# gitMasterLiujiahui/AlphaZero-Gomoku

Hardware: AMD Instinct MI355X
Metric: self-play moves/sec at 200 sims/move, 15x15 board, 1/2/4/8 MI355X (higher is better)
Workload: dtype f16x3 (fp32-equivalent split, f32 accumulate); tree forward: root children as a delta of the root's fp32 accumulators, within 2e-5 of the full forward and 1e-4 of the reference (tests/test_gpu_pvdelta.py)

## Files before the change

### alphazero-gomoku_amd/csrc/gz_pvdg.hip

```cpp
#include <hip/hip_runtime.h>

#include <cstdlib>

#include "gz_internal.h"
#include "gz_pvtree.h"

using namespace gzpv;

namespace {

using namespace gzc;

constexpr int NTD = 256;
#ifndef GZ_DG_NTE
#define GZ_DG_NTE 1
#endif
__host__ __device__ constexpr int dg_s(int L) { return 2 * L + 3; }
__host__ __device__ constexpr int dg_ss(int L) { return dg_s(L) * dg_s(L); }
__host__ __device__ constexpr int dg_so(int L) { return 2 * L + 5; }

__host__ __device__ constexpr int dgk_g(int L) { return L == 0 ? 6 : (L == 1 ? 3 : (L == 2 ? 2 : 1)); }
__host__ __device__ constexpr int dgk_npos(int L) { return (dgk_g(L) * dg_ss(L) + 1 + 15) & ~15; }
struct K {
    static constexpr int C = 6;
    __host__ __device__ static constexpr int g(int L) { return dgk_g(L); }
    static constexpr int NPASS = 1 + C / 3 + C / 2 + C;
    __host__ __device__ static constexpr int pass_of(int L, int gi) {
        return L == 0 ? 0 : (L == 1 ? 1 + gi / 3 : (L == 2 ? 3 + 3 * (gi / 2) : 4 + 3 * (gi / 2) + (gi & 1)));
    }
    __host__ __device__ static constexpr int npos(int L) { return dgk_npos(L); }
    static constexpr int MAXNPOS = 112;
    static constexpr int NMAX = 12;
    static constexpr int ROWS = NMAX * 16;
    static constexpr int GB = 2;
    static constexpr int WPS = 2;
    static constexpr int NKEY = 36;
    static constexpr int IN = 0;
    static constexpr int IN_BYTES = 32 * MAXNPOS * 16;
    static constexpr int COL = 32 * dgk_npos(0) * 16;
    static constexpr int HP = IN + IN_BYTES;
    static constexpr int HP_BYTES = dgk_g(3) * 4 * 3 * 121 * 4;
    static constexpr int ROWT = HP + HP_BYTES;
    static constexpr int MASK = ROWT + NPASS * ROWS * 4;
    static constexpr int HIST = MASK + NPASS * 16 * 4;
    static constexpr int U = HIST + 2 * NPASS * NKEY * 4;
    static constexpr int CST = U + C * 128;
    static constexpr int CST_FLOATS = 4 * 128 + 3 * 128 + 4;
    static constexpr int POS = CST + CST_FLOATS * 4;
    static constexpr int LDS = POS + 16;
};
static_assert(dgk_npos(0) <= K::MAXNPOS && dgk_npos(1) <= K::MAXNPOS && dgk_npos(2) == K::MAXNPOS &&
                  dgk_npos(3) <= K::MAXNPOS, "image");
static_assert(K::LDS * K::WPS <= 160 * 1024, "LDS budget");
static_assert(K::COL + K::C * 1024 <= K::IN_BYTES, "im2col behind the y1 image");
static_assert(dgk_g(0) * dg_so(0) * dg_so(0) <= K::ROWS && dgk_g(1) * dg_so(1) * dg_so(1) <= K::ROWS &&
                  dgk_g(2) * dg_so(2) * dg_so(2) <= K::ROWS && dgk_g(3) * dg_so(3) * dg_so(3) <= K::ROWS, "rows");
static_assert(K::C % 6 == 0 && dgk_g(3) == 1, "passes; one x2 node per pass (the record prefetch)");
static_assert(K::C == 6 && dgk_g(1) == 3 && dgk_g(2) == 2, "pass order (K::pass_of, dg_pass_of): 2 x1 triples, 3 y2 pairs");

__host__ __device__ constexpr int scr_sq(int map, int node) {
    return (map == 0 ? 9 * node : (map == 2 ? 54 + 49 * node : (map == 1 ? 348 + (node >= 3 ? 25 * (node - 3) : 0) : 348))) * 256;
}
constexpr int SCR_HALVES = (348 + 81) * 256;
static_assert(348 + 3 * 25 <= 348 + 81 && 54 + 49 * 6 == 348, "scratch regions");

struct DgUnit {
    const _Float16* gm;
    const float* pre;
    _Float16* own;
    _Float16* patch;
    int leaf, base, cell, pad0;
    int sq[4];
    uint32_t board[16];
};
static_assert(sizeof(DgUnit) == 128, "unit size");

struct DgArgs {
    const int32_t* cinfo;
    const float* W;
    const uint32_t* boards;
    const int32_t* meta;
    const int32_t* pslot;
    const _Float16* maps;
    const float* pres;
    _Float16* patches;
    float* hbuf;
    int32_t* tiles;
    int32_t* queue;
};

#ifdef GZ_PVDG_STAMPS
__device__ unsigned long long gz_pvdg_stamps[16];
__device__ unsigned long long gz_pvdg_stamps_n[1];
using DgStamp = PhaseStamp<gz_pvdg_stamps>;
#else
using DgStamp = PhaseStamp<nullptr>;
#endif

#define GZ_GLB __attribute__((address_space(1)))
#ifdef GZ_DG_CHK
__device__ unsigned long long gz_dg_chk[16];
__device__ const char* gz_dg_lo;
__device__ const char* gz_dg_hi;
__device__ __forceinline__ const void* dg_chk(const void* p, int code) {
    if ((const char*)p < gz_dg_lo || (const char*)p >= gz_dg_hi) {
        atomicAdd(&gz_dg_chk[code], 1ull);
        return gz_dg_lo;
    }
    return p;
}
#define DG_CHK(p, code) dg_chk((p), (code))
#else
#define DG_CHK(p, code) (p)
#endif
template <class T>
__device__ __forceinline__ T gld(const void* p) {
    return *(const GZ_GLB T*)DG_CHK(p, 0);
}
template <class T>
__device__ __forceinline__ void gst(void* p, const T& v) {
    *(GZ_GLB T*)DG_CHK(p, 1) = v;
}

__device__ __forceinline__ int set_rank(int b) {
    return b == 7 ? 0 : (b == 3 ? 1 : (b == 1 ? 2 : (b == 6 ? 3 : (b == 2 ? 4 : 5))));
}

__device__ __forceinline__ void dg_rows_all(char* lds, const DgUnit* U, int ng, int tid) {
    uint32_t* hist = (uint32_t*)(lds + K::HIST);
    uint32_t* starts = hist + K::NPASS * K::NKEY;
    uint32_t* rt0 = (uint32_t*)(lds + K::ROWT);
    uint32_t* mk0 = (uint32_t*)(lds + K::MASK);
    constexpr int N0 = 25, N1 = 49, N2 = 81, N3 = 121;
    const int o1 = ng * N0, o2 = o1 + ng * N1, o3 = o2 + ng * N2, tot = o3 + ng * N3;
    constexpr int PER = (K::C * (N0 + N1 + N2 + N3) + NTD - 1) / NTD;
    int kk[PER], rank[PER];
    uint32_t ent[PER];
#pragma unroll
    for (int i = 0; i < PER; i++) {
        const int c = tid + i * NTD;
        kk[i] = -1;
        rank[i] = 0;
        ent[i] = 0;
        if (c >= tot) continue;
        const int L = c < o1 ? 0 : (c < o2 ? 1 : (c < o3 ? 2 : 3));
        const int SO = 2 * L + 5, RO = L + 2, RIN = L + 1;
        const int cl = c - (L == 0 ? 0 : (L == 1 ? o1 : (L == 2 ? o2 : o3)));
        const int gi = cl / (SO * SO), j = cl - gi * (SO * SO), dy = j / SO - RO, dx = j - (j / SO) * SO - RO;
        const int cell = U[gi].cell, cr = cell / BN, cc = cell - (cell / BN) * BN;
        const int pr = cr + dy, pc = cc + dx;
        if (pr < 0 || pr >= BN || pc < 0 || pc >= BN) continue;
        int ty = 0, tx = 0;
#pragma unroll
        for (int d = -1; d <= 1; d++) {
            const int qy = dy + d, qx = dx + d;
            if (qy >= -RIN && qy <= RIN && cr + qy >= 0 && cr + qy < BN) ty |= 1 << (d + 1);
            if (qx >= -RIN && qx <= RIN && cc + qx >= 0 && cc + qx < BN) tx |= 1 << (d + 1);
        }
        if (!ty || !tx) continue;
        uint32_t m = 0;
#pragma unroll
        for (int a = 0; a < 3; a++)
            if ((ty >> a) & 1) m |= (uint32_t)tx << (3 * a);
        const int gl = L == 0 ? 0 : (L == 1 ? 3 : (L == 2 ? 2 : 1));
        const int p = K::pass_of(L, gi), u0 = L == 0 ? 0 : (gi / gl) * gl;
        kk[i] = p * K::NKEY + set_rank(ty) * 6 + set_rank(tx);
        ent[i] = (uint32_t)(gi - u0) | ((uint32_t)(dy + RO) << 4) | ((uint32_t)(dx + RO) << 8) | (m << 12) | (1u << 21);
        rank[i] = (int)atomicAdd(&hist[kk[i]], 1u);
    }
    __syncthreads();
    {
        const int w = tid >> 6, ln = tid & 63;
        for (int p = w; p < K::NPASS; p += NTD / 64) {
            const uint32_t v = ln < K::NKEY ? hist[p * K::NKEY + ln] : 0u;
            uint32_t x = v;
#pragma unroll
            for (int d = 1; d < 64; d <<= 1) {
                const uint32_t y = __shfl_up(x, d);
                if (ln >= d) x += y;
            }
            if (ln < K::NKEY) {
                starts[p * K::NKEY + ln] = x - v;
                hist[p * K::NKEY + ln] = 0u;
            }
            if (ln == 63) mk0[p * 16 + 9] = x;
        }
    }
    __syncthreads();
#pragma unroll
    for (int i = 0; i < PER; i++)
        if (kk[i] >= 0) rt0[(kk[i] / K::NKEY) * K::ROWS + starts[kk[i]] + rank[i]] = ent[i];
    for (int e = tid; e < K::NPASS * K::ROWS; e += NTD)
        if ((uint32_t)(e % K::ROWS) >= mk0[(e / K::ROWS) * 16 + 9]) rt0[e] = 0u;
    __syncthreads();
    {
        const int w = tid >> 6, ln = tid & 63;
        for (int p = w; p < K::NPASS; p += NTD / 64) {
            const uint32_t* rt = rt0 + p * K::ROWS;
            uint32_t tm = 0;
            if (ln < K::NMAX)
#pragma unroll
                for (int k = 0; k < 16; k++) tm |= (rt[ln * 16 + k] >> 12) & 0x1ffu;
            int exec = 0;
#pragma unroll
            for (int t = 0; t < 9; t++) {
                const uint64_t b = __ballot((tm >> t) & 1u);
                if (ln == 0) mk0[p * 16 + t] = (uint32_t)b;
                exec += __popcll(b);
            }
            if (ln == 0) mk0[p * 16 + 10] = (uint32_t)exec;
        }
    }
}

template <int NT, int L>
__device__ __forceinline__ void dg_kloop(const char* lds, const uint32_t (&ri)[K::NMAX], const uint32_t* mk,
                                         const _Float16* __restrict__ Wf, int nt0, int lane,
                                         f32x4 (&acc)[2][K::NMAX]) {
    constexpr int S = dg_s(L), NPOS = K::npos(L), CQ = 4, KS = 9 * CQ;
    constexpr int CQB = 4 * NPOS * 16, PLB = 16 * NPOS * 16, ZIDX = NPOS - 1;
    constexpr int KS_BYTES = 8 * 64 * 8 * 2, LO_BYTES = KS * KS_BYTES, RING = 4;
    const int lb = K::IN + (lane >> 4) * NPOS * 16;
    const __amdgpu_buffer_rsrc_t wr = __builtin_amdgcn_make_buffer_rsrc((void*)Wf, 0, 0x7fffffff, 0x00020000);
    const int wo = (nt0 * 64 + lane) * 16;
    auto wload = [&](int ks, int n, int lo) -> h8 {
        return __builtin_bit_cast(h8, __builtin_amdgcn_raw_buffer_load_b128(wr, wo, ks * KS_BYTES + n * 1024 + lo * LO_BYTES, 0));
    };
    auto addr = [&](int tap, uint32_t r) -> int {
        const int toff = (tap / 3 - 1) * S + (tap - (tap / 3) * 3 - 1);
        const bool v = (r >> (16 + tap)) & 1u;
        return lb + (v ? (int)(r & 0xffffu) - 32 + toff : ZIDX) * 16;
    };
    h8 b[RING][2][2];
#pragma unroll
    for (int c = 0; c < 2; c++)
#pragma unroll
        for (int n = 0; n < 2; n++) {
            b[c][n][0] = wload(c, n, 0);
            b[c][n][1] = wload(c, n, 1);
        }
    f32x4 c[2][NT];
#pragma unroll
    for (int n = 0; n < 2; n++)
#pragma unroll
        for (int m = 0; m < NT; m++) c[n][m] = acc[n][m];
    int ad[NT];
#pragma unroll
    for (int m = 0; m < NT; m++) ad[m] = addr(0, ri[m]);
    h8 fh[2][2], fl[2][2];
#pragma unroll
    for (int k2 = 0; k2 < 2; k2++) {
        fh[0][k2] = *(const h8*)(lds + ad[0] + k2 * CQB);
        fl[0][k2] = *(const h8*)(lds + ad[0] + k2 * CQB + PLB);
    }
#pragma unroll 1
    for (int tap = 0; tap < 9; tap++) {
        const uint32_t tm = (uint32_t)__builtin_amdgcn_readfirstlane((int)mk[tap]);
#pragma unroll
        for (int h = 0; h < 2; h++) {
            {
                const int ksr = tap * CQ + 2 * h + 2;
                const int kn = ksr < KS ? ksr : ksr - KS;
#pragma unroll
                for (int k2 = 0; k2 < 2; k2++)
#pragma unroll
                    for (int n = 0; n < 2; n++) {
                        b[(2 * h + 2 + k2) & 3][n][0] = wload(kn + k2, n, 0);
                        b[(2 * h + 2 + k2) & 3][n][1] = wload(kn + k2, n, 1);
                    }
            }
#pragma unroll
            for (int m = 0; m < NT; m++) {
                const int pm = m & 1, pn = (m + 1) & 1;
                int na;
                if (m + 1 < NT) na = ad[m + 1] + 2 * h * CQB;
                else na = h == 0 ? ad[0] + 2 * CQB : ad[0];
#pragma unroll
                for (int k2 = 0; k2 < 2; k2++) {
                    fh[pn][k2] = *(const h8*)(lds + na + k2 * CQB);
                    fl[pn][k2] = *(const h8*)(lds + na + k2 * CQB + PLB);
                }
                if (h == 1) ad[m] = addr(tap + 1, ri[m]);
                if ((tm >> m) & 1u) {
#pragma unroll
                    for (int k2 = 0; k2 < 2; k2++) {
                        const int sl = 2 * h + k2;
                        const h8 ah = fh[pm][k2], al = fl[pm][k2];
#pragma unroll
                        for (int n = 0; n < 2; n++) c[n][m] = __builtin_amdgcn_mfma_f32_16x16x32_f16(b[sl][n][0], ah, c[n][m], 0, 0, 0);
#pragma unroll
                        for (int n = 0; n < 2; n++) c[n][m] = __builtin_amdgcn_mfma_f32_16x16x32_f16(b[sl][n][1], ah, c[n][m], 0, 0, 0);
#pragma unroll
                        for (int n = 0; n < 2; n++) c[n][m] = __builtin_amdgcn_mfma_f32_16x16x32_f16(b[sl][n][0], al, c[n][m], 0, 0, 0);
                    }
                }
            }
        }
    }
#pragma unroll
    for (int n = 0; n < 2; n++)
#pragma unroll
        for (int m = 0; m < NT; m++) acc[n][m] = c[n][m];
}

struct H4x2 {
    h4 h, l;
};
__device__ __forceinline__ float h2f(const H4x2& x, int r) { return (float)x.h[r] + (float)x.l[r]; }
__device__ __forceinline__ void put_hl(_Float16* p, int plane_halves, const f32x4& v) {
    h4 hi, lo;
#pragma unroll
    for (int r = 0; r < 4; r++) {
        const _Float16 h = (_Float16)v[r];
        hi[r] = h;
        lo[r] = (_Float16)(v[r] - (float)h);
    }
    gst<h4>(p, hi);
    gst<h4>(p + plane_halves, lo);
}
__device__ __forceinline__ void put_hl_lds(_Float16* p, int plane_halves, const f32x4& v) {
    h4 hi, lo;
#pragma unroll
    for (int r = 0; r < 4; r++) {
        const _Float16 h = (_Float16)v[r];
        hi[r] = h;
        lo[r] = (_Float16)(v[r] - (float)h);
    }
    *(h4*)p = hi;
    *(h4*)(p + plane_halves) = lo;
}

template <int L>
__device__ __forceinline__ void dg_epilogue(char* lds, const DgUnit* U, const uint32_t* rt, int np, int lane,
                                            const f32x4 (&acc)[2][K::NMAX], int nt, int ldsg) {
    constexpr int RO = L + 2, SO = dg_so(L), SSO = SO * SO;
    constexpr bool SKIP = L == 1 || L == 3;
    constexpr int RS = L == 1 ? 1 : 3, SK = 2 * RS + 1, SSK = SK * SK;
    constexpr int GB = K::GB, NGRP = (K::NMAX + GB - 1) / GB, ST = 2;
    float* hpart = (float*)(lds + K::HP);
    const int q = lane >> 4, li = lane & 15;
    const float* cst = (const float*)(lds + K::CST);
    f32x4 es[2], e0[2], e1[2], ev[2];
#pragma unroll
    for (int n = 0; n < 2; n++) {
        const int ch0 = (2 * np + n) * 16 + 4 * q;
        es[n] = *(const f32x4*)(cst + L * 128 + ch0);
        if (L == 3) {
            e0[n] = *(const f32x4*)(cst + 512 + ch0);
            e1[n] = *(const f32x4*)(cst + 640 + ch0);
            ev[n] = *(const f32x4*)(cst + 768 + ch0);
        }
    }
    f32x4 z[ST][GB][2];
    H4x2 dk[ST][GB][2];
    uint32_t ent[ST][GB];
    auto loads = [&](int grp, int st) {
#pragma unroll
        for (int j = 0; j < GB; j++) {
            const int m = grp * GB + j;
            if (m >= K::NMAX) break;
            const uint32_t e = rt[m * 16 + li];
            ent[st][j] = e;
            const int gi = e & 15, dy = (int)((e >> 4) & 15) - RO, dx = (int)((e >> 8) & 15) - RO;
            const DgUnit& u = U[gi];
            const int cell = u.cell, cr = cell / BN, cc = cell - (cell / BN) * BN;
            const bool v = (e >> 21) & 1u;
            const int pos = v ? (cr + dy) * BN + (cc + dx) : 0;
            const bool near = SKIP && v && iabs(dy) <= RS && iabs(dx) <= RS;
            const int sidx = near ? (dy + RS) * SK + (dx + RS) : 0;
#pragma unroll
            for (int n = 0; n < 2; n++) {
                const int ch0 = (2 * np + n) * 16 + 4 * q;
                z[st][j][n] = gld<f32x4>(u.pre + L * PV_PRE_FLOATS + pos * CH + ch0);
                if (SKIP) {
                    const _Float16* p = u.own + u.sq[L - 1] + ((ch0 >> 3) * SSK + sidx) * 8 + (ch0 & 7);
                    dk[st][j][n] = H4x2{gld<h4>(p), gld<h4>(p + 16 * SSK * 8)};
                }
            }
        }
    };
#pragma unroll
    for (int grp = 0; grp < ST - 1; grp++)
        if (grp * GB < nt) loads(grp, grp);
#pragma unroll
    for (int grp = 0; grp < NGRP; grp++) {
        if (grp * GB >= nt) break;
        const int st = grp % ST;
        if ((grp + ST - 1) * GB < nt) loads(grp + ST - 1, (grp + ST - 1) % ST);
#pragma unroll
        for (int j = 0; j < GB; j++) {
            const int m = grp * GB + j;
            if (m >= K::NMAX) break;
            const uint32_t e = ent[st][j];
            const bool v = (e >> 21) & 1u;
            const int gi = e & 15, dy = (int)((e >> 4) & 15) - RO, dx = (int)((e >> 8) & 15) - RO;
            const bool near = SKIP && iabs(dy) <= RS && iabs(dx) <= RS;
            const int oidx = (dy + RO) * SO + (dx + RO);
            float s0 = 0.f, s1 = 0.f, sv = 0.f;
#pragma unroll
            for (int n = 0; n < 2; n++) {
                const int ch0 = (2 * np + n) * 16 + 4 * q;
                f32x4 y, d;
#pragma unroll
                for (int r = 0; r < 4; r++) {
                    const float zr = z[st][j][n][r];
                    float tc = __builtin_fmaf(acc[n][m][r], es[n][r], zr);
                    if (SKIP) tc += near ? h2f(dk[st][j][n], r) : 0.f;
                    tc = tc > 0.f ? tc : 0.f;
                    if (L == 3) {
                        s0 = __builtin_fmaf(e0[n][r], tc, s0);
                        s1 = __builtin_fmaf(e1[n][r], tc, s1);
                        sv = __builtin_fmaf(ev[n][r], tc, sv);
                    } else {
                        y[r] = tc;
                        d[r] = tc - (zr > 0.f ? zr : 0.f);
                    }
                }
                if (L < 3 && v) {
                    const DgUnit& u = U[gi];
                    const int o = PATCH_OFF[L + 1] + ((ch0 >> 3) * SSO + oidx) * 8 + (ch0 & 7);
                    if (gi < ldsg) {
                        constexpr int NPN = K::npos(L + 1 < 4 ? L + 1 : 3), SSN = SSO;
                        put_hl_lds((_Float16*)(lds + K::IN) + ((ch0 >> 3) * NPN + gi * SSN + oidx) * 8 + (ch0 & 7),
                                   16 * NPN * 8, d);
                    } else {
                        put_hl(u.own + u.sq[L + 1] + ((ch0 >> 3) * SSO + oidx) * 8 + (ch0 & 7), 16 * SSO * 8, d);
                    }
                    if (u.patch) put_hl(u.patch + o, 16 * SSO * 8, y);
                }
            }
            if (L == 3) {
                s0 += __shfl_xor(s0, 16);
                s1 += __shfl_xor(s1, 16);
                sv += __shfl_xor(sv, 16);
                s0 += __shfl_xor(s0, 32);
                s1 += __shfl_xor(s1, 32);
                sv += __shfl_xor(sv, 32);
                if (lane < 16 && v) {
                    float* h = hpart + ((gi * 4 + np) * 3) * 121 + oidx;
                    h[0] = s0;
                    h[121] = s1;
                    h[242] = sv;
                }
            }
        }
    }
}

constexpr int REC_K = (HSTRIDE + NTD - 1) / NTD;
__device__ __forceinline__ void dg_record_load(const DgUnit& u, const float* __restrict__ hbuf, float (&rec)[REC_K],
                                               int tid) {
    const float* src = (const float*)DG_CHK(hbuf + (size_t)u.base * HSTRIDE, 3);
#pragma unroll
    for (int k = 0; k < REC_K; k++) {
        const int j = tid + k * NTD;
        rec[k] = j < HSTRIDE ? src[j] : 0.f;
    }
}
__device__ __forceinline__ void dg_record(const DgUnit& u, int g, const float* bias, float* __restrict__ hbuf,
                                          const float* hpart, const float (&rec)[REC_K], int tid) {
    const int cr = u.cell / BN, cc = u.cell - (u.cell / BN) * BN;
    float* h = (float*)DG_CHK(hbuf + (size_t)u.leaf * HSTRIDE, 4);
#pragma unroll
    for (int k = 0; k < REC_K; k++) {
        const int j = tid + k * NTD;
        if (j >= HSTRIDE) break;
        float v = rec[k];
        int pos = -1, which = 0;
        if (j < POS) {
            pos = j;
        } else if (j < 2 * POS) {
            pos = j - POS;
            which = 1;
        } else if (j >= HV_OFF && j < HV_OFF + POS) {
            pos = j - HV_OFF;
            which = 2;
        }
        if (pos >= 0) {
            const int dy = pos / BN - cr, dx = pos % BN - cc;
            if (iabs(dy) <= 5 && iabs(dx) <= 5) {
                const int idx = (dy + 5) * 11 + (dx + 5);
                float a = bias[which];
#pragma unroll
                for (int w = 0; w < 4; w++) a += hpart[((g * 4 + w) * 3 + which) * 121 + idx];
                v = a;
            }
        }
        h[j] = v;
    }
}

template <int L>
__device__ __forceinline__ void dg_fill(char* lds, const DgUnit* U, int g, int tid) {
    constexpr int SS = dg_ss(L), NPOS = K::npos(L), NB = (NPOS + 63) / 64;
    const int lane = tid & 63, wave = tid >> 6;
#pragma unroll
    for (int blk = 0; blk < NB; blk++) {
        const int idx = blk * 64 + lane;
        const _Float16* src = (const _Float16*)gz_tree_zero16;
        int stride = 0;
        if (idx < g * SS) {
            const int gi = idx / SS, j = idx - gi * SS;
            src = U[gi].own + U[gi].sq[L] + j * 8;
            stride = SS * 8;
        }
        char* dst = lds + K::IN + blk * 64 * 16;
        if (idx < NPOS) {
#pragma unroll
            for (int k = 0; k < 8; k++) {
                const int pc = wave * 8 + k;
                __builtin_amdgcn_global_load_lds((glb_void_t*)DG_CHK(src + pc * stride, 2), (lds_void_t*)(dst + pc * NPOS * 16),
                                                 16, 0, 0);
            }
        }
    }
}

__device__ __forceinline__ void dg_col(_Float16* col, const DgUnit* U, int ng, int tid) {
    for (int e = tid; e < ng * 512; e += NTD) {
        const int g = e >> 9, row = (e >> 5) & 15, k = e & 31;
        const DgUnit& u = U[g];
        const int cr = u.cell / BN, cc = u.cell - (u.cell / BN) * BN;
        const int r0 = cr > 0 ? cr - 1 : 0, r1 = cr < BN - 1 ? cr + 1 : BN - 1;
        const int c0 = cc > 0 ? cc - 1 : 0, c1 = cc < BN - 1 ? cc + 1 : BN - 1, wr = c1 - c0 + 1;
        _Float16 v = (_Float16)0.f;
        if (row < (r1 - r0 + 1) * wr && k < 27) {
            const int pr = r0 + row / wr, pc = c0 + row % wr;
            const int tap = k / 3, cin = k % 3;
            const int rr = pr + tap / 3 - 1, c2 = pc + tap % 3 - 1;
            if (rr >= 0 && rr < BN && c2 >= 0 && c2 < BN) {
                const int bit = rr * 16 + c2;
                const uint32_t bl = (u.board[bit >> 5] >> (bit & 31)) & 1u, wh = (u.board[8 + (bit >> 5)] >> (bit & 31)) & 1u;
                v = (_Float16)(float)(cin == 0 ? bl : (cin == 1 ? wh : 1u - (bl | wh)));
            }
        }
        col[e] = v;
    }
}

__device__ __forceinline__ void dg_conv0(char* lds, const _Float16* col, const DgUnit* U, int ng,
                                         const float* __restrict__ W, int np, int lane) {
    constexpr int NPOS = K::npos(0);
    const int li = lane & 15, q = lane >> 4;
    h8 wh[2], wl[2];
    f32x4 ws[2], wt[2];
#pragma unroll
    for (int n = 0; n < 2; n++) {
        const int nt = 2 * np + n, ch0 = nt * 16 + 4 * q;
        const _Float16* wf = (const _Float16*)(W + F16_C0) + ((size_t)nt * 64 + lane) * 8;
        wh[n] = *(const h8*)wf;
        wl[n] = *(const h8*)(wf + 8 * 64 * 8);
        ws[n] = *(const f32x4*)(W + C0_S + ch0);
        wt[n] = *(const f32x4*)(W + C0_T + ch0);
    }
    _Float16* in = (_Float16*)(lds + K::IN);
    h4 rxh[K::C][2], rxl[K::C][2];
#pragma unroll
    for (int g = 0; g < K::C; g++) {
        const DgUnit& u = U[g < ng ? g : 0];
        const int cr = u.cell / BN, cc = u.cell - (u.cell / BN) * BN;
        const int r0 = cr > 0 ? cr - 1 : 0, r1 = cr < BN - 1 ? cr + 1 : BN - 1;
        const int c0 = cc > 0 ? cc - 1 : 0, c1 = cc < BN - 1 ? cc + 1 : BN - 1, wr = c1 - c0 + 1;
        const bool rowok = li < (r1 - r0 + 1) * wr;
        const int pr = rowok ? r0 + li / wr : cr, pc = rowok ? c0 + li % wr : cc, pos = pr * BN + pc;
#pragma unroll
        for (int n = 0; n < 2; n++) {
            const int ch0 = (2 * np + n) * 16 + 4 * q;
            const _Float16* rp = u.gm + ((ch0 >> 3) * 256 + pos) * 8 + (ch0 & 7);
            rxh[g][n] = gld<h4>(rp);
            rxl[g][n] = gld<h4>(rp + PV_MAP_PLANE);
        }
    }
#pragma unroll
    for (int g = 0; g < K::C; g++) {
        if (g >= ng) break;
        const h8 a = *(const h8*)(col + g * 512 + li * 32 + 8 * q);
        const DgUnit& u = U[g];
        const int cr = u.cell / BN, cc = u.cell - (u.cell / BN) * BN;
        const int r0 = cr > 0 ? cr - 1 : 0, r1 = cr < BN - 1 ? cr + 1 : BN - 1;
        const int c0 = cc > 0 ? cc - 1 : 0, c1 = cc < BN - 1 ? cc + 1 : BN - 1, wr = c1 - c0 + 1;
        const bool rowok = li < (r1 - r0 + 1) * wr;
        const int pr = rowok ? r0 + li / wr : cr, pc = rowok ? c0 + li % wr : cc;
        const int idx = (pr - cr + 1) * 3 + (pc - cc + 1);
#pragma unroll
        for (int n = 0; n < 2; n++) {
            const int ch0 = (2 * np + n) * 16 + 4 * q;
            f32x4 acc = zero4();
            acc = __builtin_amdgcn_mfma_f32_16x16x32_f16(wh[n], a, acc, 0, 0, 0);
            acc = __builtin_amdgcn_mfma_f32_16x16x32_f16(wl[n], a, acc, 0, 0, 0);
            if (rowok) {
                const h4 rh = rxh[g][n], rl = rxl[g][n];
                f32x4 y, d;
#pragma unroll
                for (int r = 0; r < 4; r++) {
                    float t = __builtin_fmaf(acc[r], ws[n][r], wt[n][r]);
                    t = t > 0.f ? t : 0.f;
                    y[r] = t;
                    d[r] = t - ((float)rh[r] + (float)rl[r]);
                }
                put_hl_lds(in + ((ch0 >> 3) * NPOS + g * 9 + idx) * 8 + (ch0 & 7), 16 * NPOS * 8, d);
                const int o = PATCH_OFF[0] + ((ch0 >> 3) * 9 + idx) * 8 + (ch0 & 7);
                put_hl(u.own + u.sq[0] + o, 16 * 9 * 8, d);
                if (u.patch) put_hl(u.patch + o, 16 * 9 * 8, y);
            }
        }
    }
}

template <int L>
__device__ __forceinline__ void dg_pass(const char* lds, const uint32_t* rt, const uint32_t* mk,
                                        const float* __restrict__ W, int np, int lane, f32x4 (&acc)[2][K::NMAX], int nt) {
    constexpr int RIN = L + 1, RO = L + 2, S = dg_s(L), SS = dg_ss(L);
    const int li = lane & 15;
    uint32_t ri[K::NMAX];
#pragma unroll
    for (int m = 0; m < K::NMAX; m++) {
        const uint32_t e = rt[m * 16 + li];
        const int gi = e & 15, dy = (int)((e >> 4) & 15) - RO, dx = (int)((e >> 8) & 15) - RO;
        const int base = gi * SS + (dy + RIN) * S + (dx + RIN) + 32;
        ri[m] = (e >> 21) & 1u ? ((uint32_t)base & 0xffffu) | (((e >> 12) & 0x1ffu) << 16) : 0u;
    }
#pragma unroll
    for (int n = 0; n < 2; n++)
#pragma unroll
        for (int m = 0; m < K::NMAX; m++) acc[n][m] = zero4();
    const _Float16* Wf = (const _Float16*)(W + F16_RES0 + L * F16_STRIDE);
#if GZ_DG_NTE
    constexpr int MT = (dgk_g(L) * dg_so(L) * dg_so(L) + 15) / 16, MTE = (MT + 1) & ~1;
    static_assert(MTE <= K::NMAX, "tiles");
    const int nte = (nt + 1) & ~1;
    if (nte <= 2)
        dg_kloop<2, L>(lds, ri, mk, Wf, 2 * np, lane, acc);
    else if (nte == 4)
        dg_kloop<4, L>(lds, ri, mk, Wf, 2 * np, lane, acc);
    else if (nte == 6 || MTE <= 6)
        dg_kloop<6 < MTE ? 6 : MTE, L>(lds, ri, mk, Wf, 2 * np, lane, acc);
    else if (nte == 8 || MTE <= 8)
        dg_kloop<8 < MTE ? 8 : MTE, L>(lds, ri, mk, Wf, 2 * np, lane, acc);
    else if (nte == 10 || MTE <= 10)
        dg_kloop<10 < MTE ? 10 : MTE, L>(lds, ri, mk, Wf, 2 * np, lane, acc);
    else
        dg_kloop<MTE, L>(lds, ri, mk, Wf, 2 * np, lane, acc);
#else
    if (nt <= 4)
        dg_kloop<4, L>(lds, ri, mk, Wf, 2 * np, lane, acc);
    else if (nt <= 8)
        dg_kloop<8, L>(lds, ri, mk, Wf, 2 * np, lane, acc);
    else
        dg_kloop<K::NMAX, L>(lds, ri, mk, Wf, 2 * np, lane, acc);
#endif
}

__device__ __forceinline__ void dg_pass_of(int p, int ng, int& L, int& u0, int& g) {
    if (p < 3) {
        L = p == 0 ? 0 : 1;
        u0 = p == 0 ? 0 : (p - 1) * 3;
    } else {
        const int k = (p - 3) / 3, r = p - 3 - 3 * k;
        L = r == 0 ? 2 : 3;
        u0 = 2 * k + (r == 2 ? 1 : 0);
    }
    g = ng - u0 < K::g(L) ? ng - u0 : K::g(L);
    if (L == 0) u0 = 0, g = ng;
}

__global__ __launch_bounds__(NTD, K::WPS) void pv_dg_kernel(DgArgs A, _Float16* __restrict__ scratch,
                                                           const int32_t* __restrict__ list,
                                                           const int32_t* __restrict__ list_count) {
    __shared__ __attribute__((aligned(16))) char lds[K::LDS];
    DgUnit* const U = (DgUnit*)(lds + K::U);
    const int count = *list_count;
    const int nx = gridDim.x >= 8 ? 8 : 1;
    const int xcd = blockIdx.x % nx, per = gridDim.x / nx, k = blockIdx.x / nx;
    if (k >= per) return;
    const int xchunk = (count + nx - 1) / nx;
    int q = 0, claim = 0;
    if (threadIdx.x == 0) claim = atomicAdd(A.queue + xcd, K::C);
    _Float16* myscr = scratch + (size_t)blockIdx.x * SCR_HALVES;
    const int tid = threadIdx.x, lane = tid & 63;
    const int wave = __builtin_amdgcn_readfirstlane(tid >> 6), np = wave;
    const float* W = A.W;
    for (int i = tid; i < K::NPASS * K::NKEY; i += NTD) ((uint32_t*)(lds + K::HIST))[i] = 0u;
    {
        float* cst = (float*)(lds + K::CST);
        for (int i = tid; i < K::CST_FLOATS; i += NTD) {
            float v;
            if (i < 512) v = W[RES0 + (i >> 7) * RES_STRIDE + RES_S + (i & 127)];
            else if (i < 768) v = W[P_W + (i - 512)];
            else if (i < 896) v = W[V_W + (i - 768)];
            else v = i == 896 ? W[P_B] : (i == 897 ? W[P_B + 1] : (i == 898 ? W[V_B] : 0.f));
            cst[i] = v;
        }
    }
    DgStamp st;
    for (;;) {
        __syncthreads();
        if (threadIdx.x == 0) {
            int pb = count, pe = count;
            for (;;) {
                const int qx = (xcd + q) % nx, xb = qx * xchunk, xe = xb + xchunk < count ? xb + xchunk : count;
                if (xb + claim < xe) {
                    pb = xb + claim, pe = xe;
                    claim = atomicAdd(A.queue + qx, K::C);
                    break;
                }
                if (++q == nx) break;
                claim = atomicAdd(A.queue + (xcd + q) % nx, K::C);
            }
            ((int*)(lds + K::POS))[0] = pb;
            ((int*)(lds + K::POS))[1] = pe;
        }
        __syncthreads();
        const int pos = ((const int*)(lds + K::POS))[0], xe = ((const int*)(lds + K::POS))[1];
        if (pos >= xe) break;
        const int ng = xe - pos < K::C ? xe - pos : K::C;
        if (wave == 0 && lane < ng) {
            const int b = list[pos + lane];
            DgUnit u;
            const int ci = A.cinfo[b];
            const int o = (ci >> 8) & 0x3fffff;
            u.gm = A.maps + (size_t)o * 4 * PV_MAP_HALVES;
            u.pre = A.pres + (size_t)o * 4 * PV_PRE_FLOATS;
            u.own = myscr;
            u.sq[0] = scr_sq(0, lane);
            u.sq[1] = scr_sq(1, lane);
            u.sq[2] = scr_sq(2, lane);
            u.sq[3] = scr_sq(3, lane);
            const int ps = A.pslot[b];
            u.patch = ps >= 0 ? A.patches + (size_t)ps * PATCH_HALVES : nullptr;
            u.leaf = b;
            u.base = A.meta[b];
            u.cell = ci & 0xff;
            u.pad0 = 0;
#pragma unroll
            for (int w = 0; w < 16; w++) u.board[w] = A.boards[(size_t)b * 16 + w];
            U[lane] = u;
        }
        __syncthreads();
        {
            int t = tid;
            asm volatile("" : "+v"(t));
            dg_col((_Float16*)(lds + K::COL), U, ng, t);
            constexpr int NPOS0 = K::npos(0);
            const int z0 = ng * 9;
            for (int e = t; e < 32 * (NPOS0 - z0); e += NTD) {
                const int pc = e / (NPOS0 - z0), idx = z0 + e % (NPOS0 - z0);
                *(uint4*)(lds + K::IN + (pc * NPOS0 + idx) * 16) = make_uint4(0u, 0u, 0u, 0u);
            }
            __syncthreads();
            const float* Wp = W;
            asm volatile("" : "+s"(Wp));
            dg_conv0(lds, (const _Float16*)(lds + K::COL), U, ng, Wp, np, t & 63);
            dg_rows_all(lds, U, ng, t);
            __syncthreads();
#ifdef GZ_DG_CHK
            for (int e = tid; e < K::NPASS * K::ROWS; e += NTD) {
                const int pp = e / K::ROWS;
                int L_, u0_, g_;
                dg_pass_of(pp, ng, L_, u0_, g_);
                const uint32_t tot = ((const uint32_t*)(lds + K::MASK))[pp * 16 + 9];
                const uint32_t en = ((const uint32_t*)(lds + K::ROWT))[e];
                if ((uint32_t)(e % K::ROWS) < tot && (!((en >> 21) & 1u) || (int)(en & 15) >= g_))
                    atomicAdd(&gz_dg_chk[8], 1ull);
                if ((uint32_t)(e % K::ROWS) >= tot && en != 0u) atomicAdd(&gz_dg_chk[9], 1ull);
            }
            if (tid < K::C && (U[tid].cell < 0 || U[tid].cell >= 225) && tid < ng) atomicAdd(&gz_dg_chk[10], 1ull);
#endif
        }
        st(0);
#ifdef GZ_PVDG_STAMPS
        if (blockIdx.x == 0 && threadIdx.x == 0) atomicAdd(&gz_pvdg_stamps_n[0], (unsigned long long)ng);
#endif
        for (int p = 0; p < K::NPASS; p++) {
            int L, u0, g;
            dg_pass_of(p, ng, L, u0, g);
            if (g <= 0) continue;
            const uint32_t* rt = (const uint32_t*)(lds + K::ROWT) + p * K::ROWS;
            const uint32_t* mk = (const uint32_t*)(lds + K::MASK) + p * 16;
            const int nrows = (int)mk[9], nt = (nrows + 15) >> 4;
            if (A.tiles && tid == 0) atomicAdd(A.tiles, (int)mk[10]);
            const float* Wp = W;
            int t = tid;
            asm volatile("" : "+s"(Wp), "+v"(t));
#ifdef GZ_DG_CHK
            for (int e = tid; e < K::ROWS; e += NTD) {
                const uint32_t en = rt[e];
                if ((uint32_t)e < (uint32_t)nrows && (!((en >> 21) & 1u) || (int)(en & 15) >= g))
                    atomicAdd(&gz_dg_chk[11 + (L > 1 ? 1 : 0)], 1ull);
            }
#endif
            f32x4 acc[2][K::NMAX];
            if (L == 0) dg_pass<0>(lds, rt, mk, Wp, np, t & 63, acc, nt);
            else if (L == 1) dg_pass<1>(lds, rt, mk, Wp, np, t & 63, acc, nt);
            else if (L == 2) dg_pass<2>(lds, rt, mk, Wp, np, t & 63, acc, nt);
            else dg_pass<3>(lds, rt, mk, Wp, np, t & 63, acc, nt);
            st(2 + L);
            __syncthreads();
            st(6);
            int q = p + 1, L2 = 0, v0 = 0, g2 = 0;
            for (; q < K::NPASS; q++) {
                dg_pass_of(q, ng, L2, v0, g2);
                if (g2 > 0) break;
            }
            const bool more = q < K::NPASS;
            const int ldsg = more && L2 == L + 1 && v0 == u0 && (L == 0 || L == 2) ? g2 : 0;
            const bool to_lds = ldsg > 0;
            if (L == 0) dg_epilogue<0>(lds, U + u0, rt, np, t & 63, acc, nt, ldsg);
            else if (L == 1) dg_epilogue<1>(lds, U + u0, rt, np, t & 63, acc, nt, 0);
            else if (L == 2) dg_epilogue<2>(lds, U + u0, rt, np, t & 63, acc, nt, ldsg);
            else dg_epilogue<3>(lds, U + u0, rt, np, t & 63, acc, nt, 0);
            if (to_lds) {
                const int NPN = L == 0 ? K::npos(1) : K::npos(3), z0 = ldsg * (L == 0 ? dg_ss(1) : dg_ss(3));
                for (int e = t; e < 32 * (NPN - z0); e += NTD) {
                    const int pc = e / (NPN - z0), idx = z0 + e % (NPN - z0);
                    *(uint4*)(lds + K::IN + (pc * NPN + idx) * 16) = make_uint4(0u, 0u, 0u, 0u);
                }
            }
            st(7 + L);
            const bool reads_mine = more && !to_lds && L2 == L + 1 && v0 < u0 + g && u0 < v0 + g2;
            if (reads_mine) asm volatile("s_waitcnt vmcnt(0)" ::: "memory");
            if (reads_mine || L == 3) __syncthreads();
            st(11);
            if (more && !to_lds) {
                if (L2 == 1) dg_fill<1>(lds, U + v0, g2, t);
                else if (L2 == 2) dg_fill<2>(lds, U + v0, g2, t);
                else if (L2 == 3) dg_fill<3>(lds, U + v0, g2, t);
            }
            if (L == 3) {
                float rec[REC_K];
                dg_record_load(U[u0], A.hbuf, rec, t);
                dg_record(U[u0], 0, (const float*)(lds + K::CST) + 896, A.hbuf, (const float*)(lds + K::HP), rec, t);
                asm volatile("s_waitcnt vmcnt(2)" ::: "memory");
            } else {
                asm volatile("s_waitcnt vmcnt(0)" ::: "memory");
            }
            st(12);
            __syncthreads();
            st(13);
        }
    }
}

}

int gz_internal_tree_delta(const TreeWs& t, const float* d_weights, const uint32_t* d_boards, const int32_t* d_meta,
                           int grid, void* stream) {
    DgArgs A{t.cinfo, d_weights, d_boards, d_meta, t.pslot, t.maps, t.pres, t.patches, t.hbuf,
             t.ctr + CTR_TILES, t.ctr + CTR_DG_QUEUE};
    static_assert(K::WPS * SCR_HALVES <= PV_SCRATCH_PATCHES * PATCH_HALVES, "scratch");
#ifdef GZ_PVDG_STAMPS
    static const int wps = std::getenv("GZ_PVDG_WPS") && std::getenv("GZ_PVDG_WPS")[0] == '1' ? 1 : K::WPS;
#else
    constexpr int wps = K::WPS;
#endif
#ifdef GZ_DG_CHK
    {
        const char* lo = (const char*)t.hbuf;
        const char* hi = (const char*)(t.scratch + (size_t)grid * PV_SCRATCH_PATCHES * PATCH_HALVES);
        hipMemcpyToSymbolAsync(HIP_SYMBOL(gz_dg_lo), &lo, sizeof(lo), 0, hipMemcpyHostToDevice, (hipStream_t)stream);
        hipMemcpyToSymbolAsync(HIP_SYMBOL(gz_dg_hi), &hi, sizeof(hi), 0, hipMemcpyHostToDevice, (hipStream_t)stream);
    }
#endif
    pv_dg_kernel<<<grid * wps, NTD, 0, (hipStream_t)stream>>>(A, t.scratch, t.children, t.ctr + CTR_CHILDREN);
    return gz_check_launch("tree delta");
}

#ifdef GZ_PVDG_STAMPS
extern "C" int gz_pvdg_stamps_read(unsigned long long* out, int reset) {
    if (hipMemcpyFromSymbol(out, HIP_SYMBOL(gz_pvdg_stamps), 16 * sizeof(unsigned long long)) != hipSuccess) return -1;
    if (hipMemcpyFromSymbol(out + 16, HIP_SYMBOL(gz_pvdg_stamps_n), sizeof(unsigned long long)) != hipSuccess) return -1;
    if (reset) {
        unsigned long long z[16] = {0};
        if (hipMemcpyToSymbol(HIP_SYMBOL(gz_pvdg_stamps), z, sizeof(z)) != hipSuccess) return -1;
        if (hipMemcpyToSymbol(HIP_SYMBOL(gz_pvdg_stamps_n), z, sizeof(z[0])) != hipSuccess) return -1;
    }
    return 0;
}
#endif

#ifdef GZ_DG_CHK
extern "C" int gz_pvdg_chk_read(unsigned long long* out) {
    if (hipDeviceSynchronize() != hipSuccess) return -1;
    return hipMemcpyFromSymbol(out, HIP_SYMBOL(gz_dg_chk), 16 * sizeof(unsigned long long)) == hipSuccess ? 0 : -1;
}
#endif
```

Measured before the change: 37150.

## Remap MFMA output channels so each lane owns 8 contiguous channels

```diff
diff --git a/alphazero-gomoku_amd/csrc/gz_dgclass.h b/alphazero-gomoku_amd/csrc/gz_dgclass.h
--- /dev/null
+++ b/alphazero-gomoku_amd/csrc/gz_dgclass.h
@@ -0,0 +1,32 @@
+#pragma once
+
+#ifdef __HIPCC__
+#define GZ_DGCLASS_FN __host__ __device__ constexpr
+#else
+#define GZ_DGCLASS_FN constexpr
+#endif
+
+GZ_DGCLASS_FN int dg_set_rank(int b) {
+    return b == 1 ? 0 : (b == 3 ? 1 : (b == 7 ? 2 : (b == 6 ? 3 : (b == 4 ? 4 : 5))));
+}
+GZ_DGCLASS_FN bool dg_set_valid(int b) { return b == 1 || b == 3 || b == 7 || b == 6 || b == 4 || b == 2; }
+
+GZ_DGCLASS_FN int dg_class_rank(int ty, int tx) {
+    const int ry = dg_set_rank(ty), rx = dg_set_rank(tx);
+    return ry * 6 + ((ry & 1) ? 5 - rx : rx);
+}
+
+GZ_DGCLASS_FN bool dg_class_rank_is_permutation() {
+    unsigned long long seen = 0;
+    for (int ty = 1; ty < 8; ty++)
+        for (int tx = 1; tx < 8; tx++) {
+            if (!dg_set_valid(ty) || !dg_set_valid(tx)) continue;
+            const int k = dg_class_rank(ty, tx);
+            if (k < 0 || k >= 36 || ((seen >> k) & 1ull)) return false;
+            seen |= 1ull << k;
+        }
+    return seen == (1ull << 36) - 1ull;
+}
+static_assert(dg_class_rank_is_permutation(), "the 36 valid (ty, tx) pairs map onto 0..35 exactly once");
+
+#undef GZ_DGCLASS_FN
diff --git a/alphazero-gomoku_amd/csrc/gz_pvdg.hip b/alphazero-gomoku_amd/csrc/gz_pvdg.hip
--- a/alphazero-gomoku_amd/csrc/gz_pvdg.hip
+++ b/alphazero-gomoku_amd/csrc/gz_pvdg.hip
@@ -2,6 +2,7 @@
 
 #include <cstdlib>
 
+#include "gz_dgclass.h"
 #include "gz_internal.h"
 #include "gz_pvtree.h"
 
@@ -122,9 +123,13 @@
     *(GZ_GLB T*)DG_CHK(p, 1) = v;
 }
 
-__device__ __forceinline__ int set_rank(int b) {
-    return b == 7 ? 0 : (b == 3 ? 1 : (b == 1 ? 2 : (b == 6 ? 3 : (b == 2 ? 4 : 5))));
-}
+__device__ __forceinline__ int dg_ch0(int np, int q, int n) { return 32 * np + 8 * q + 4 * n; }
+__device__ __forceinline__ int dg_wfrag(int np, int lane) {
+    const int i = lane & 15;
+    return (2 * np + (i >> 3)) * 64 + ((lane & 48) | (8 * ((i >> 2) & 1) + (i & 3)));
+}
+constexpr int DG_WFRAG_N = 4;
+
 
 __device__ __forceinline__ void dg_rows_all(char* lds, const DgUnit* U, int ng, int tid) {
     uint32_t* hist = (uint32_t*)(lds + K::HIST);
@@ -164,7 +169,7 @@
             if ((ty >> a) & 1) m |= (uint32_t)tx << (3 * a);
         const int gl = L == 0 ? 0 : (L == 1 ? 3 : (L == 2 ? 2 : 1));
         const int p = K::pass_of(L, gi), u0 = L == 0 ? 0 : (gi / gl) * gl;
-        kk[i] = p * K::NKEY + set_rank(ty) * 6 + set_rank(tx);
+        kk[i] = p * K::NKEY + dg_class_rank(ty, tx);
         ent[i] = (uint32_t)(gi - u0) | ((uint32_t)(dy + RO) << 4) | ((uint32_t)(dx + RO) << 8) | (m << 12) | (1u << 21);
         rank[i] = (int)atomicAdd(&hist[kk[i]], 1u);
     }
@@ -222,9 +227,9 @@
     constexpr int KS_BYTES = 8 * 64 * 8 * 2, LO_BYTES = KS * KS_BYTES, RING = 4;
     const int lb = K::IN + (lane >> 4) * NPOS * 16;
     const __amdgpu_buffer_rsrc_t wr = __builtin_amdgcn_make_buffer_rsrc((void*)Wf, 0, 0x7fffffff, 0x00020000);
-    const int wo = (nt0 * 64 + lane) * 16;
+    const int wo = dg_wfrag(nt0 >> 1, lane) * 16;
     auto wload = [&](int ks, int n, int lo) -> h8 {
-        return __builtin_bit_cast(h8, __builtin_amdgcn_raw_buffer_load_b128(wr, wo, ks * KS_BYTES + n * 1024 + lo * LO_BYTES, 0));
+        return __builtin_bit_cast(h8, __builtin_amdgcn_raw_buffer_load_b128(wr, wo, ks * KS_BYTES + n * DG_WFRAG_N * 16 + lo * LO_BYTES, 0));
     };
     auto addr = [&](int tap, uint32_t r) -> int {
         const int toff = (tap / 3 - 1) * S + (tap - (tap / 3) * 3 - 1);
@@ -303,31 +308,29 @@
         for (int m = 0; m < NT; m++) acc[n][m] = c[n][m];
 }
 
-struct H4x2 {
-    h4 h, l;
+struct H8x2 {
+    h8 h, l;
 };
-__device__ __forceinline__ float h2f(const H4x2& x, int r) { return (float)x.h[r] + (float)x.l[r]; }
-__device__ __forceinline__ void put_hl(_Float16* p, int plane_halves, const f32x4& v) {
-    h4 hi, lo;
-#pragma unroll
-    for (int r = 0; r < 4; r++) {
-        const _Float16 h = (_Float16)v[r];
-        hi[r] = h;
-        lo[r] = (_Float16)(v[r] - (float)h);
-    }
-    gst<h4>(p, hi);
-    gst<h4>(p + plane_halves, lo);
-}
-__device__ __forceinline__ void put_hl_lds(_Float16* p, int plane_halves, const f32x4& v) {
-    h4 hi, lo;
-#pragma unroll
-    for (int r = 0; r < 4; r++) {
-        const _Float16 h = (_Float16)v[r];
-        hi[r] = h;
-        lo[r] = (_Float16)(v[r] - (float)h);
-    }
-    *(h4*)p = hi;
-    *(h4*)(p + plane_halves) = lo;
+__device__ __forceinline__ float h2f(const H8x2& x, int r) { return (float)x.h[r] + (float)x.l[r]; }
+__device__ __forceinline__ H8x2 split_hl(const f32x4 (&v)[2]) {
+    H8x2 o;
+#pragma unroll
+    for (int n = 0; n < 2; n++)
+#pragma unroll
+        for (int r = 0; r < 4; r++) {
+            const _Float16 h = (_Float16)v[n][r];
+            o.h[4 * n + r] = h;
+            o.l[4 * n + r] = (_Float16)(v[n][r] - (float)h);
+        }
+    return o;
+}
+__device__ __forceinline__ void put_hl(_Float16* p, int plane_halves, const H8x2& x) {
+    gst<h8>(p, x.h);
+    gst<h8>(p + plane_halves, x.l);
+}
+__device__ __forceinline__ void put_hl_lds(_Float16* p, int plane_halves, const H8x2& x) {
+    *(h8*)p = x.h;
+    *(h8*)(p + plane_halves) = x.l;
 }
 
 template <int L>
@@ -338,12 +341,12 @@
     constexpr int RS = L == 1 ? 1 : 3, SK = 2 * RS + 1, SSK = SK * SK;
     constexpr int GB = K::GB, NGRP = (K::NMAX + GB - 1) / GB, ST = 2;
     float* hpart = (float*)(lds + K::HP);
-    const int q = lane >> 4, li = lane & 15;
+    const int q = lane >> 4, li = lane & 15, cg = 4 * np + q;
     const float* cst = (const float*)(lds + K::CST);
     f32x4 es[2], e0[2], e1[2], ev[2];
 #pragma unroll
     for (int n = 0; n < 2; n++) {
-        const int ch0 = (2 * np + n) * 16 + 4 * q;
+        const int ch0 = dg_ch0(np, q, n);
         es[n] = *(const f32x4*)(cst + L * 128 + ch0);
         if (L == 3) {
             e0[n] = *(const f32x4*)(cst + 512 + ch0);
@@ -352,7 +355,7 @@
         }
     }
     f32x4 z[ST][GB][2];
-    H4x2 dk[ST][GB][2];
+    H8x2 dk[ST][GB];
     uint32_t ent[ST][GB];
     auto loads = [&](int grp, int st) {
 #pragma unroll
@@ -369,13 +372,11 @@
             const bool near = SKIP && v && iabs(dy) <= RS && iabs(dx) <= RS;
             const int sidx = near ? (dy + RS) * SK + (dx + RS) : 0;
 #pragma unroll
-            for (int n = 0; n < 2; n++) {
-                const int ch0 = (2 * np + n) * 16 + 4 * q;
-                z[st][j][n] = gld<f32x4>(u.pre + L * PV_PRE_FLOATS + pos * CH + ch0);
-                if (SKIP) {
-                    const _Float16* p = u.own + u.sq[L - 1] + ((ch0 >> 3) * SSK + sidx) * 8 + (ch0 & 7);
-                    dk[st][j][n] = H4x2{gld<h4>(p), gld<h4>(p + 16 * SSK * 8)};
-                }
+            for (int n = 0; n < 2; n++)
+                z[st][j][n] = gld<f32x4>(u.pre + L * PV_PRE_FLOATS + pos * CH + dg_ch0(np, q, n));
+            if (SKIP) {
+                const _Float16* p = u.own + u.sq[L - 1] + (cg * SSK + sidx) * 8;
+                dk[st][j] = H8x2{gld<h8>(p), gld<h8>(p + 16 * SSK * 8)};
             }
         }
     };
@@ -397,37 +398,35 @@
             const bool near = SKIP && iabs(dy) <= RS && iabs(dx) <= RS;
             const int oidx = (dy + RO) * SO + (dx + RO);
             float s0 = 0.f, s1 = 0.f, sv = 0.f;
+            f32x4 y[2], d[2];
 #pragma unroll
             for (int n = 0; n < 2; n++) {
-                const int ch0 = (2 * np + n) * 16 + 4 * q;
-                f32x4 y, d;
 #pragma unroll
                 for (int r = 0; r < 4; r++) {
                     const float zr = z[st][j][n][r];
                     float tc = __builtin_fmaf(acc[n][m][r], es[n][r], zr);
-                    if (SKIP) tc += near ? h2f(dk[st][j][n], r) : 0.f;
+                    if (SKIP) tc += near ? h2f(dk[st][j], 4 * n + r) : 0.f;
                     tc = tc > 0.f ? tc : 0.f;
                     if (L == 3) {
                         s0 = __builtin_fmaf(e0[n][r], tc, s0);
                         s1 = __builtin_fmaf(e1[n][r], tc, s1);
                         sv = __builtin_fmaf(ev[n][r], tc, sv);
                     } else {
-                        y[r] = tc;
-                        d[r] = tc - (zr > 0.f ? zr : 0.f);
+                        y[n][r] = tc;
+                        d[n][r] = tc - (zr > 0.f ? zr : 0.f);
                     }
                 }
-                if (L < 3 && v) {
-                    const DgUnit& u = U[gi];
-                    const int o = PATCH_OFF[L + 1] + ((ch0 >> 3) * SSO + oidx) * 8 + (ch0 & 7);
-                    if (gi < ldsg) {
-                        constexpr int NPN = K::npos(L + 1 < 4 ? L + 1 : 3), SSN = SSO;
-                        put_hl_lds((_Float16*)(lds + K::IN) + ((ch0 >> 3) * NPN + gi * SSN + oidx) * 8 + (ch0 & 7),
-                                   16 * NPN * 8, d);
-                    } else {
-                        put_hl(u.own + u.sq[L + 1] + ((ch0 >> 3) * SSO + oidx) * 8 + (ch0 & 7), 16 * SSO * 8, d);
-                    }
-                    if (u.patch) put_hl(u.patch + o, 16 * SSO * 8, y);
+            }
+            if (L < 3 && v) {
+                const DgUnit& u = U[gi];
+                const H8x2 dd = split_hl(d);
+                if (gi < ldsg) {
+                    constexpr int NPN = K::npos(L + 1 < 4 ? L + 1 : 3), SSN = SSO;
+                    put_hl_lds((_Float16*)(lds + K::IN) + (cg * NPN + gi * SSN + oidx) * 8, 16 * NPN * 8, dd);
+                } else {
+                    put_hl(u.own + u.sq[L + 1] + (cg * SSO + oidx) * 8, 16 * SSO * 8, dd);
                 }
+                if (u.patch) put_hl(u.patch + PATCH_OFF[L + 1] + (cg * SSO + oidx) * 8, 16 * SSO * 8, split_hl(y));
             }
             if (L == 3) {
                 s0 += __shfl_xor(s0, 16);
@@ -509,7 +508,8 @@
 #pragma unroll
             for (int k = 0; k < 8; k++) {
                 const int pc = wave * 8 + k;
-                __builtin_amdgcn_global_load_lds((glb_void_t*)DG_CHK(src + pc * stride, 2), (lds_void_t*)(dst + pc * NPOS * 16),
+                const _Float16* sp = src + pc * stride;
+                __builtin_amdgcn_global_load_lds((glb_void_t*)(stride ? DG_CHK(sp, 2) : sp), (lds_void_t*)(dst + pc * NPOS * 16),
                                                  16, 0, 0);
             }
         }
@@ -541,20 +541,20 @@
 __device__ __forceinline__ void dg_conv0(char* lds, const _Float16* col, const DgUnit* U, int ng,
                                          const float* __restrict__ W, int np, int lane) {
     constexpr int NPOS = K::npos(0);
-    const int li = lane & 15, q = lane >> 4;
+    const int li = lane & 15, q = lane >> 4, cg = 4 * np + q;
     h8 wh[2], wl[2];
     f32x4 ws[2], wt[2];
 #pragma unroll
     for (int n = 0; n < 2; n++) {
-        const int nt = 2 * np + n, ch0 = nt * 16 + 4 * q;
-        const _Float16* wf = (const _Float16*)(W + F16_C0) + ((size_t)nt * 64 + lane) * 8;
+        const int ch0 = dg_ch0(np, q, n);
+        const _Float16* wf = (const _Float16*)(W + F16_C0) + (size_t)(dg_wfrag(np, lane) + n * DG_WFRAG_N) * 8;
         wh[n] = *(const h8*)wf;
         wl[n] = *(const h8*)(wf + 8 * 64 * 8);
         ws[n] = *(const f32x4*)(W + C0_S + ch0);
         wt[n] = *(const f32x4*)(W + C0_T + ch0);
     }
     _Float16* in = (_Float16*)(lds + K::IN);
-    h4 rxh[K::C][2], rxl[K::C][2];
+    h8 rxh[K::C], rxl[K::C];
 #pragma unroll
     for (int g = 0; g < K::C; g++) {
         const DgUnit& u = U[g < ng ? g : 0];
@@ -563,13 +563,9 @@
         const int c0 = cc > 0 ? cc - 1 : 0, c1 = cc < BN - 1 ? cc + 1 : BN - 1, wr = c1 - c0 + 1;
         const bool rowok = li < (r1 - r0 + 1) * wr;
         const int pr = rowok ? r0 + li / wr : cr, pc = rowok ? c0 + li % wr : cc, pos = pr * BN + pc;
-#pragma unroll
-        for (int n = 0; n < 2; n++) {
-            const int ch0 = (2 * np + n) * 16 + 4 * q;
-            const _Float16* rp = u.gm + ((ch0 >> 3) * 256 + pos) * 8 + (ch0 & 7);
-            rxh[g][n] = gld<h4>(rp);
-            rxl[g][n] = gld<h4>(rp + PV_MAP_PLANE);
-        }
+        const _Float16* rp = u.gm + (cg * 256 + pos) * 8;
+        rxh[g] = gld<h8>(rp);
+        rxl[g] = gld<h8>(rp + PV_MAP_PLANE);
     }
 #pragma unroll
     for (int g = 0; g < K::C; g++) {
@@ -582,27 +578,26 @@
         const bool rowok = li < (r1 - r0 + 1) * wr;
         const int pr = rowok ? r0 + li / wr : cr, pc = rowok ? c0 + li % wr : cc;
         const int idx = (pr - cr + 1) * 3 + (pc - cc + 1);
+        f32x4 y[2], d[2];
 #pragma unroll
         for (int n = 0; n < 2; n++) {
-            const int ch0 = (2 * np + n) * 16 + 4 * q;
             f32x4 acc = zero4();
             acc = __builtin_amdgcn_mfma_f32_16x16x32_f16(wh[n], a, acc, 0, 0, 0);
             acc = __builtin_amdgcn_mfma_f32_16x16x32_f16(wl[n], a, acc, 0, 0, 0);
-            if (rowok) {
-                const h4 rh = rxh[g][n], rl = rxl[g][n];
-                f32x4 y, d;
-#pragma unroll
-                for (int r = 0; r < 4; r++) {
-                    float t = __builtin_fmaf(acc[r], ws[n][r], wt[n][r]);
-                    t = t > 0.f ? t : 0.f;
-                    y[r] = t;
-                    d[r] = t - ((float)rh[r] + (float)rl[r]);
-                }
-                put_hl_lds(in + ((ch0 >> 3) * NPOS + g * 9 + idx) * 8 + (ch0 & 7), 16 * NPOS * 8, d);
-                const int o = PATCH_OFF[0] + ((ch0 >> 3) * 9 + idx) * 8 + (ch0 & 7);
-                put_hl(u.own + u.sq[0] + o, 16 * 9 * 8, d);
-                if (u.patch) put_hl(u.patch + o, 16 * 9 * 8, y);
-            }
+#pragma unroll
+            for (int r = 0; r < 4; r++) {
+                float t = __builtin_fmaf(acc[r], ws[n][r], wt[n][r]);
+                t = t > 0.f ? t : 0.f;
+                y[n][r] = t;
+                d[n][r] = t - ((float)rxh[g][4 * n + r] + (float)rxl[g][4 * n + r]);
+            }
+        }
+        if (rowok) {
+            const H8x2 dd = split_hl(d);
+            put_hl_lds(in + (cg * NPOS + g * 9 + idx) * 8, 16 * NPOS * 8, dd);
+            const int o = PATCH_OFF[0] + (cg * 9 + idx) * 8;
+            put_hl(u.own + u.sq[0] + o, 16 * 9 * 8, dd);
+            if (u.patch) put_hl(u.patch + o, 16 * 9 * 8, split_hl(y));
         }
     }
 }
```

Result: faster. 38670 (median of 6 runs) (+4.1%).
